# szpajder/dumpvdl2

Hardware: AMD Instinct MI355X
Metric: IQ MS/s demodulated end-to-end (higher is better)
Workload: dtype f32

## Files before the change

dumpvdl2_amd/csrc/debug_hooks.inc:

```

static bool hip_ok(hipError_t e) { return e == hipSuccess; }
template<typename T> static bool dbg_up(const DevBuf<T> &d, const void *src, size_t bytes) { return hip_ok(hipMemcpy(d, src, bytes, hipMemcpyHostToDevice)); }
template<typename T> static bool dbg_up(const DevBuf<T> &d, const void *src) { return dbg_up(d, src, d.bytes()); }
template<typename T> static bool dbg_fill(const DevBuf<T> &d, int v) { return hip_ok(hipMemset(d, v, d.bytes())); }
template<typename T> static bool dbg_down(void *dst, const DevBuf<T> &d, size_t bytes) { return hip_ok(hipMemcpy(dst, d, bytes, hipMemcpyDeviceToHost)); }
template<typename T> static bool dbg_down(void *dst, const DevBuf<T> &d) { return dbg_down(dst, d, d.bytes()); }
static bool dbg_tables(const DevBuf<Tables> &d) { auto tab = std::make_unique<Tables>(); build_tables(*tab); return dbg_up(d, tab.get()); }

template<int K> static int prof_read(const void *symbol, unsigned long long *out, int reset) {
	unsigned long long h[64][K];
	if(hipMemcpyFromSymbol(h, symbol, sizeof h) != hipSuccess) return -3;
	for(int k = 0; k < K; k++) { out[k] = 0; for(int s = 0; s < 64; s++) out[k] += h[s][k]; }
	if(reset) { memset(h, 0, sizeof h); if(hipMemcpyToSymbol(symbol, h, sizeof h) != hipSuccess) return -3; }
	return 0;
}

extern "C" {

int vdl2hip_debug_live_resources(long long out[3]) {
	if(!out) return VDL2HIP_E_INVAL;
	for(int i = 0; i < 3; i++) out[i] = hostmem::g_live[i].load();
	return VDL2HIP_OK;
}

int vdl2hip_debug_option(vdl2hip_ctx *c, const char *name, long value) {
	if(!c || !name) return VDL2HIP_E_INVAL;
	OnDevice dev_guard(c);
	int r = collect_pending(c);
	if(r != VDL2HIP_OK && r != VDL2HIP_E_OVERFLOW) return r;
	if(strcmp(name, "no_fuse") == 0) { c->fuse_k2 = value == 0; return VDL2HIP_OK; }
	if(strcmp(name, "force_timeout") == 0) { c->debug_force_timeout = value != 0; return VDL2HIP_OK; }
	if(strcmp(name, "force_mismatch") == 0) { c->debug_force_mismatch = value != 0; return VDL2HIP_OK; }
	if(strcmp(name, "walk_ahead_below") == 0) { c->walk_ahead_below = (double)value; c->walk_ahead_auto = true; return VDL2HIP_OK; }
	if(strcmp(name, "mark_cap") == 0) { if(value < 0 || value > (long long)kDeferScansMax) return VDL2HIP_E_INVAL; c->debug_mark_cap = (uint32_t)value; return VDL2HIP_OK; }
	if(strcmp(name, "walk_ahead") == 0) { if(value != 0 && value != 1) return VDL2HIP_E_INVAL; c->walk_ahead = (int)value; c->walk_ahead_auto = false; return VDL2HIP_OK; }
	if(strcmp(name, "exact_tier") == 0) { if(value != 0 && value != 1) return VDL2HIP_E_INVAL; c->debug_exact_tier = (int)value; return VDL2HIP_OK; }
	if(strcmp(name, "screen_all") == 0) { c->debug_screen_all = value != 0; return VDL2HIP_OK; }
	if(strcmp(name, "force_again") == 0) { c->debug_force_again = value != 0; return VDL2HIP_OK; }
	if(strcmp(name, "referee") == 0) { if(value && !c->d_refhist) return VDL2HIP_E_INVAL; c->referee = value != 0; return VDL2HIP_OK; }
	if(strcmp(name, "ref_warm") == 0) { if(value < 0 || value > c->ref_T - 4096) return VDL2HIP_E_INVAL; c->ref_warm = value; return VDL2HIP_OK; }
	return VDL2HIP_E_INVAL;
}

int vdl2hip_debug_exact_window_many(vdl2hip_ctx *c, uint32_t chan, int64_t n_lo, int64_t n_hi, uint32_t count, int64_t stride, float *ms) {
	if(!c || !c->d_refhist || chan >= (uint32_t)c->C || c->feed_no == 0 || count == 0 || count > 65536) return VDL2HIP_E_INVAL;
	OnDevice dev_guard(c);
	int r = collect_pending(c);
	if(r != VDL2HIP_OK && r != VDL2HIP_E_OVERFLOW) return r;
	DevBuf<int> d_out; std::vector<int> h(count, 0);
	if(!hip_ok(d_out.alloc(count))) return VDL2HIP_E_NOMEM;
	Event e0, e1;
	if(!hip_ok(e0.ensure()) || !hip_ok(e1.ensure())) return VDL2HIP_E_DEVICE;
	hipExtLaunchKernelGGL(k_ref_probe, dim3(count), dim3(64), 0, c->streams.front, e0, e1, 0, c->d_ref[(c->feed_no - 1) % kSlots].get(), (int)chan, c->C, n_lo, n_hi, stride, d_out.get());
	if(!hip_ok(hipStreamSynchronize(c->streams.front)) || !dbg_down(h.data(), d_out)) return VDL2HIP_E_DEVICE;
	if(ms) { float t = 0.f; (void)hipEventElapsedTime(&t, e0, e1); *ms = t; }
	int n = 0; for(int v : h) n += v;
	return n;
}
int vdl2hip_debug_scan_multi2(vdl2hip_ctx *c, const int32_t *chan, const int64_t *lo, const int64_t *hi, uint32_t count, int with_retry, float *ms) {
	if(!c || !c->d_refhist || c->feed_no == 0 || count == 0 || count > 65536 || !chan || !lo || !hi) return VDL2HIP_E_INVAL;
	OnDevice dev_guard(c);
	int r = collect_pending(c);
	if(r != VDL2HIP_OK && r != VDL2HIP_E_OVERFLOW) return r;
	std::vector<ScanReq> h(count);
	for(uint32_t i = 0; i < count; i++) { if(chan[i] < 0 || chan[i] >= c->C) return VDL2HIP_E_INVAL; h[i] = ScanReq{ chan[i], REF_CANDIDATE, lo[i], hi[i] }; }
	DevBuf<ScanReq> d_sq, d_rt; DevBuf<uint32_t> d_n;
	if(!hip_ok(d_sq.alloc(count)) || !hip_ok(d_n.alloc(2)) || !hip_ok(d_rt.alloc(kRetryScans))) return VDL2HIP_E_NOMEM;
	uint32_t before[8] = {0}, after[8] = {0};
	const uint32_t nn[2] = { count, 0u };
	Event e0, e1;
	if(!hip_ok(e0.ensure()) || !hip_ok(e1.ensure()) || !dbg_up(d_sq, h.data()) || !dbg_up(d_n, nn) || !dbg_down(before, c->d_refstats, sizeof before)) return VDL2HIP_E_DEVICE;
	RefChan *ref = c->d_ref[(c->feed_no - 1) % kSlots];
	launch_scans(c, c->streams.front, ref, 0xfffeu, d_sq, nullptr, d_n, count, c->k_total, with_retry ? d_rt.get() : nullptr, d_n + 1, e0, e1);
	if(!hip_ok(hipStreamSynchronize(c->streams.front)) || !dbg_down(after, c->d_refstats, sizeof after)) return VDL2HIP_E_DEVICE;
	if(ms) { float t = 0.f; (void)hipEventElapsedTime(&t, e0, e1); *ms = t; }
	return (int)(after[0] - before[0]);
}
int vdl2hip_debug_exact_window(vdl2hip_ctx *c, uint32_t chan, int64_t n_lo, int64_t n_hi) { return vdl2hip_debug_exact_window_many(c, chan, n_lo, n_hi, 1, 0, nullptr); }

int vdl2hip_debug_u8_levels(float out[512]) {
	DevBuf<float> d;
	if(!hip_ok(d.alloc(512))) return VDL2HIP_E_NOMEM;
	hipLaunchKernelGGL(k_u8_level_probe, dim3(1), dim3(256), 0, 0, d);
	return dbg_down(out, d) ? VDL2HIP_OK : VDL2HIP_E_DEVICE;
}

int vdl2hip_debug_s8_levels(float out[512]) {
	DevBuf<float> d;
	if(!hip_ok(d.alloc(512))) return VDL2HIP_E_NOMEM;
// ... 466 lines not shown
```

dumpvdl2_amd/csrc/kernels.h:

```cpp
#pragma once
#include <hip/hip_runtime.h>
#include <type_traits>
#include "vdl2_core.h"
#include "design.h"

#ifndef VDL2_K1_UNROLL
#define VDL2_K1_UNROLL 5
#endif

#ifndef VDL2_K1_WAVES_PER_EU
#define VDL2_K1_WAVES_PER_EU 3
#endif

namespace vdl2 {

constexpr int kK1Unroll = VDL2_K1_UNROLL;
typedef float v2f __attribute__((ext_vector_type(2)));
typedef float v4f __attribute__((ext_vector_type(4)));

#ifndef VDL2_REF_PRIO
#define VDL2_REF_PRIO 3
#endif
#ifndef VDL2_K1_PRIO
#define VDL2_K1_PRIO 0
// ... 902 lines not shown
	const int c = blockIdx.y;
	if(k >= a.D) return;
	const BlockForm &bf = *a.bf;
	const uint32_t slot = (uint32_t)(a.k0 + k) & a.mask;
	const int seg = (int)(k / a.seglen), i = (int)(k - (int64_t)seg * a.seglen);
	if(i < kFixW) {
		cf32 v = a.y[(size_t)c * a.cap + slot];
		const float4 ts = seg ? a.seg_end[(size_t)c * a.nseg_cap + seg - 1] : a.carry_in[c];
		v.re += bf.cP[i][0] * ts.x + bf.cP[i][1] * ts.z;
		v.im += bf.cP[i][0] * ts.y + bf.cP[i][1] * ts.w;
		a.y[(size_t)c * a.cap + slot] = v;
	}
	if(k == a.D - 1) {
		const int len = i + 1;
		float4 e = a.seg_end[(size_t)c * a.nseg_cap + seg];
		if(len <= kFixW) {
			const float4 ts = seg ? a.seg_end[(size_t)c * a.nseg_cap + seg - 1] : a.carry_in[c];
			const float *Pp = bf.Ppow[len];
			e.x += Pp[0] * ts.x + Pp[1] * ts.z; e.y += Pp[0] * ts.y + Pp[1] * ts.w;
			e.z += Pp[2] * ts.x + Pp[3] * ts.z; e.w += Pp[2] * ts.y + Pp[3] * ts.w;
		}
		a.carry_out[c] = e;
	}
}

__global__ void k_carry(K1Args a, void *carry_out, uint32_t nrem) {
	const uint32_t i = threadIdx.x;
	if(i >= nrem) return;
	const int64_t s = (int64_t)(a.nlogical - nrem) + i;
	if(a.fmt == 2) {
		const uint2 *p = (s < (int64_t)a.ncarry) ? (const uint2 *)a.carry + s : (const uint2 *)a.in + (s - a.ncarry);
		((uint2 *)carry_out)[i] = *p;
	} else if(a.fmt == 1) {
		const uint32_t *p = (s < (int64_t)a.ncarry) ? (const uint32_t *)a.carry + s : (const uint32_t *)a.in + (s - a.ncarry);
		((uint32_t *)carry_out)[i] = *p;
	} else {
		const uint16_t *p = (s < (int64_t)a.ncarry) ? (const uint16_t *)a.carry + s : (const uint16_t *)a.in + (s - a.ncarry);
		((uint16_t *)carry_out)[i] = *p;
	}
}

__device__ __forceinline__ void reset_out_ctl(OutCtl *ctl, uint32_t k5_waves) {
	ctl->nbursts = 0; ctl->overflow = 0; ctl->nvalid = 0; ctl->pool_out_used = 0;
	ctl->nframes = burst_reserve_initial_frames(k5_waves); ctl->pool_used = burst_reserve_initial_pool(k5_waves);
}
__global__ void k_reset_ctl(OutCtl *ctl, uint32_t k5_waves) { reset_out_ctl(ctl, k5_waves); }

struct K3Args {
	const cf32 *y; cf32 *pf; uint64_t *cand; uint64_t *flag; const Tables *tab;
	int64_t nbase, k1;
	uint32_t cap, mask;
	int32_t wpl;
	int32_t screen_all;
	OutCtl *ctl; uint32_t k5_waves;
	RefChan *ref; RefChan refv; float max_ppm; const float *ppm_thr; int32_t ref_on; uint32_t *rq_n, *rq_flag; RefBad *rq_bad; ScanReq *pq; uint32_t pq_cap; uint32_t *rq_flag2;
};

#ifndef VDL2_K3_SHARE
#define VDL2_K3_SHARE 8
#endif
constexpr int kK3Share = VDL2_K3_SHARE, kK3Threads = 320, kK3Tile = kK3Threads * kK3Share;
static_assert(kK3Tile == kK3Threads * kK3Share && kK3Tile % 64 == 0 && kK3Threads % 10 == 0 && (kK3Tile / 64) % (kK3Threads / 64) == 0, "screen tile");

__global__ __launch_bounds__(kK3Threads) void k_sync_screen(K3Args a) {
	if(blockIdx.x == 0 && blockIdx.y == 0 && threadIdx.x == 0 && a.rq_n) a.rq_n[3] = 0u;
	__shared__ float tile[kK3Tile + 150];
	__shared__ uint8_t verdict[kK3Tile];
	const int c = blockIdx.y, tid = threadIdx.x;
	const int64_t nblk = a.nbase + (int64_t)blockIdx.x * kK3Tile;
	const cf32 *y = a.y + (size_t)c * a.cap;
	constexpr int kFull = (kK3Tile + 150) / kK3Threads, kRest = (kK3Tile + 150) % kK3Threads;
	const bool full_tile = nblk >= 150 && nblk + kK3Tile <= a.k1;
	if(full_tile) {
		const uint32_t r0 = (uint32_t)(nblk - 150) + tid;
		cf32 v[kFull + 1];
		#pragma unroll
		for(int k = 0; k <= kFull; k++) if(k < kFull || tid < kRest) v[k] = y[(r0 + kK3Threads * k) & a.mask];
		#pragma unroll
		for(int k = 0; k <= kFull; k++) if(k < kFull || tid < kRest) tile[tid + kK3Threads * k] = phase_fast(v[k]);
	} else {
		for(int j = tid; j < kK3Tile + 150; j += kK3Threads) {
			const int64_t t = nblk - 150 + j;
			tile[j] = (t < 0 || t >= a.k1) ? 0.f : phase_fast(y[(uint32_t)t & a.mask]);
		}
	}
	__syncthreads();
	const int s0 = 10 * kK3Share * (tid / 10) + tid % 10;
	constexpr int kEarlyPh = kScreenEarly + kK3Share - 1;
	float ph[kEarlyPh], d[kEarlyPh];
	#pragma unroll
	for(int k = 0; k < kEarlyPh; k++) ph[k] = tile[s0 + 10 * k];
	#pragma unroll
	for(int k = 1; k < kEarlyPh; k++) d[k] = ph[k] - ph[k - 1];
	#pragma unroll
	for(int q = 0; q < kK3Share; q++) {
		ScreenAcc acc;
		screen_begin(acc);
		screen_taps(&d[q], 1, kScreenEarly, acc);
		float ps = screen_value(acc, kScreenEarly);
		if(__any(ps < kScreenEarlyThr)) {
			float pl[kPreamble - kScreenEarly + 1], dl[kPreamble];
			#pragma unroll
			for(int j = 0; j <= kPreamble - kScreenEarly; j++) pl[j] = tile[s0 + 10 * (q + kScreenEarly - 1 + j)];
			#pragma unroll
			for(int j = 0; j < kPreamble - kScreenEarly; j++) dl[kScreenEarly + j] = pl[j + 1] - pl[j];
			screen_taps(dl, kScreenEarly, kPreamble, acc);
// ... 131 lines not shown
			#pragma unroll
			for(int k = 0; k < 4; k++) if(64 * k + lane < kSpan) e2[64 * k + lane] = ev[k];
			WAVE_SYNC();
		}
		K3B_MARK(2);
		#pragma unroll 1
		for(int round = 0; round < 2; round++) {
			const int bit = round == 0 ? lane : lane - 6;
			const bool todo = round == 0 ? ((needj >> lane) & 1ull) != 0 : (lane < 6 && ((fprevj >> lane) & 1u) && (wj << 6) + bit >= 0);
			if(todo) {
				const int i0 = bit + kBack - 150;
				float p[kPreamble];
				#pragma unroll
				for(int i = 0; i < kPreamble; i++) p[i] = ph[i0 + 10 * i];
				float pv, fv, E = 0.f, pa, pb;
				if(ref_on) sync_metric_ref(p, e2 + i0, 10, T, pv, fv, E, pa, pb, FULL);
				else { sync_metric(p, T, pv, fv); pa = pb = pv; }
				ps[6 + bit] = pv; fs[6 + bit] = fv; es[6 + bit] = E; as[6 + bit] = pa; bs[6 + bit] = pb;
			}
			K3B_MARK(3 + round);
		}
		WAVE_SYNC();
		const int64_t n = (wj << 6) + lane;
		const float p0 = ps[6 + lane], p3 = ps[3 + lane], p6 = ps[lane];
		int vd = 0;
		if(n >= 3 && n < a.k1) {
			if(!ref_on) vd = is_candidate(p3, p0) ? 1 : 0;
			else vd = ref_candidate_verdict(ref_pherr_range(p0, as[6 + lane], bs[6 + lane], es[6 + lane]), ref_pherr_range(p3, as[3 + lane], bs[3 + lane], es[3 + lane]), fs[3 + lane], es[3 + lane],
			                                ref_pherr_range(p6, as[lane], bs[lane], es[lane]), a.max_ppm, ppm_thr);
		}
		if((needj >> lane) & 1ull) a.pf[(size_t)c * a.cap + ((uint32_t)n & a.mask)] = cf32{ (vd & 2) ? -p0 : p0, fs[6 + lane] };
		const unsigned long long bits = __ballot((vd & 1) != 0);
		if(lane == 0) cand[(uint32_t)wj & wmask] = bits;
		if(a.pq) {
			const unsigned long long mk = __ballot((vd & 2) != 0 && ((needj >> lane) & 1ull) != 0);
			if(mk && lane == 0) {
				const int64_t nf = (wj << 6) + __builtin_ctzll(mk), nl = (wj << 6) + 63 - __builtin_clzll(mk);
				int64_t lo = (nf - kRefPre) & ~255ll, hi = (nl + kRefPost) | 255; if(lo < 0) lo = 0; if(hi > a.k1 - 1) hi = a.k1 - 1;
				const uint32_t i = atomicAdd(a.rq_n + 3, 1u);
				if(i < a.pq_cap) a.pq[i] = ScanReq{ c, REF_CANDIDATE, lo, hi };
			}
		}
		WAVE_SYNC();
		K3B_MARK(5);
	}
	K3B_END();
}

constexpr int kK3dEvals = 320;
constexpr int kK3dFlush = kK3dEvals - 64;
constexpr int kK3dList = kK3dFlush + 256;
constexpr int kK3dMinGroups = 2048;
constexpr int kK3dGroup = 4;
constexpr int kK3dRounds = 32;
static_assert(kK3dEvals >= 70 && kK3dEvals <= 512 && kK3dList * 70 < (1 << 20) && kK3dList < (1 << 11) && kK3dRounds * 256 <= (1 << 16),
              "tile map: 9 bits of word, 7 of position; list head: 11 bits of words, 21 of evaluations; 16 bits of word index");
#define K3D_BARRIER() do { __builtin_amdgcn_fence(__ATOMIC_RELEASE, "workgroup", "local"); __builtin_amdgcn_s_barrier(); __builtin_amdgcn_fence(__ATOMIC_ACQUIRE, "workgroup", "local"); } while(0)
template<bool FULL>
__global__ __launch_bounds__(256, 4) void k_sync_dense(K3Args a) {
	if(blockIdx.x == 0 && blockIdx.y == 0 && threadIdx.x == 0) { reset_out_ctl(a.ctl, a.k5_waves); if(a.ref) *a.ref = a.refv; if(a.rq_n) { a.rq_n[0] = 0u; a.rq_n[1] = 0u; a.rq_n[2] = 0u; a.rq_n[4] = 0u; a.rq_n[5] = 0u; a.rq_n[6] = 0u; a.rq_n[7] = 0u; } }
	if(blockIdx.x == 0 && threadIdx.x == 0 && a.rq_flag) { a.rq_flag[blockIdx.y] = 0u; a.rq_bad[blockIdx.y].n = 0u; if(a.rq_flag2) a.rq_flag2[blockIdx.y] = 0u; }
	__shared__ uint64_t s_need[kK3dList], s_cbits[kK3dList], s_mbits[kK3dList];
	__shared__ uint32_t s_end[kK3dList];
	__shared__ uint16_t s_word[kK3dList];
	__shared__ uint8_t s_fprev[kK3dList];
	__shared__ uint16_t s_map[kK3dEvals];
	__shared__ float s_res[5][kK3dEvals];
	__shared__ uint8_t s_neg[kK3dEvals];
	__shared__ uint32_t s_head, s_r1;
	__shared__ uint64_t s_flag[256 * kK3dGroup + 3];
	const int c = blockIdx.y, tid = threadIdx.x, lane = threadIdx.x & 63;
	const cf32 *y = a.y + (size_t)c * a.cap;
	const uint64_t *flag = a.flag + (size_t)c * (a.cap >> 6);
	uint64_t *cand = a.cand + (size_t)c * (a.cap >> 6);
	const uint32_t wmask = a.mask >> 6;
	const Tables &T = *a.tab;
	const bool ref_on = a.ref != nullptr && a.ref_on != 0;
	const float ppm_thr = ref_on ? a.ppm_thr[c] : 0.f;
	const int64_t w0 = a.nbase >> 6, w1 = (a.k1 + 63) >> 6;
	const int64_t wb = w0 + (int64_t)blockIdx.x * (256 * a.wpl);
	K3B_BEGIN();
	if(tid == 0) s_head = 0u;
	K3D_BARRIER();
	#pragma unroll 1
	for(int g = 0; g < a.wpl; g++) {
		if(g % kK3dGroup == 0) {
			const int ng = a.wpl - g < kK3dGroup ? a.wpl - g : kK3dGroup;
			for(int i = tid; i < 256 * ng + 3; i += 256) {
				const int64_t w = wb + 256 * g - 2 + i;
				s_flag[i] = w >= 0 && w < w1 ? flag[(uint32_t)w & wmask] : 0ull;
			}
			K3D_BARRIER();
		}
		{
			const int64_t w = wb + 256 * g + tid;
			const int fi = 256 * (g % kK3dGroup) + tid;
			uint64_t need = 0, fprev = 0, fpp = 0, f0 = 0;
			if(w < w1) {
				f0 = s_flag[fi + 2]; fprev = s_flag[fi + 1]; fpp = s_flag[fi];
				const uint64_t fnext = s_flag[fi + 3];
				need = f0 | (f0 << 3) | (f0 >> 3) | (fprev >> 61) | (fnext << 61);
				const int64_t base = w << 6;
				if(a.k1 - 3 < base + 64) {
					const int64_t lo = a.k1 - 3 - base;
					need |= lo <= 0 ? ~0ull : (~0ull << lo);
				}
				if(a.k1 < base + 64) need &= (a.k1 - base <= 0) ? 0ull : (~0ull >> (64 - (a.k1 - base)));
				if(need == 0) cand[(uint32_t)w & wmask] = 0;
			}
			const uint64_t need_prev = fprev | (fprev << 3) | (fprev >> 3) | (fpp >> 61) | (f0 << 61);
			const uint32_t fp6 = w > 0 ? (uint32_t)(need_prev >> 58) : 0u;
			const uint32_t cnt = need != 0 ? (uint32_t)__builtin_popcountll(need) + (uint32_t)__builtin_popcount(fp6) : 0u;
			const uint32_t inc = cnt << 11 | (need != 0 ? 1u : 0u);
			uint32_t incl = inc;
			#pragma unroll
			for(int d = 1; d < 64; d <<= 1) { const uint32_t o = (uint32_t)__shfl_up((int)incl, d); if(lane >= d) incl += o; }
			const uint32_t tot = (uint32_t)__shfl((int)incl, 63);
			uint32_t at = 0;
			if(lane == 0 && tot != 0) at = atomicAdd(&s_head, tot);
			at = (uint32_t)__shfl((int)at, 0) + incl - inc;
			if(need != 0) {
				const uint32_t r = at & 2047u;
				s_need[r] = need; s_fprev[r] = (uint8_t)fp6; s_word[r] = (uint16_t)(256 * g + tid); s_end[r] = (at >> 11) + cnt;
				s_cbits[r] = 0ull; s_mbits[r] = 0ull;
			}
		}
		K3D_BARRIER();
		const uint32_t head = s_head;
		K3D_BARRIER();
		const int nrec = (int)(head & 2047u);
		K3B_MARK(0);
		if((int)(head >> 11) < kK3dFlush && g + 1 < a.wpl) continue;
		K3B_COUNT(0, nrec); K3B_COUNT(1, head >> 11);
		#pragma unroll 1
		for(int r0 = 0; r0 < nrec; ) {
			const uint32_t e0 = r0 ? s_end[r0 - 1] : 0u;
			if(tid == 0) s_r1 = (uint32_t)r0 + 1u;
			K3D_BARRIER();
			{
				uint32_t best = 0;
				for(int r = r0 + 1 + tid; r < nrec && r < r0 + kK3dEvals; r += 256) if(s_end[r] - e0 <= (uint32_t)kK3dEvals) best = (uint32_t)r + 1u;
				if(best) atomicMax(&s_r1, best);
			}
			K3D_BARRIER();
			const int r1 = (int)s_r1, nev = (int)(s_end[r1 - 1] - e0);
			for(int r = r0 + tid; r < r1; r += 256) {
				uint32_t at = (r ? s_end[r - 1] : 0u) - e0;
				const uint32_t code = (uint32_t)(r - r0) << 7;
				for(uint32_t m = s_fprev[r]; m; m &= m - 1u) s_map[at++] = (uint16_t)(code | (uint32_t)__builtin_ctz(m));
				for(uint64_t m = s_need[r]; m; m &= m - 1ull) s_map[at++] = (uint16_t)(code | (6u + (uint32_t)__builtin_ctzll(m)));
			}
			K3D_BARRIER();
			K3B_MARK(1); K3B_COUNT(2, 1);
			#pragma unroll 1
			for(int s = tid; s < nev; s += 256) {
				const uint32_t code = s_map[s];
				const int64_t n = ((wb + s_word[r0 + (int)(code >> 7)]) << 6) + (int)(code & 127u) - 6;
				float p[kPreamble], e2[kPreamble];
				cf32 yt[kPreamble];
				#pragma unroll
				for(int i = 0; i < kPreamble; i++) { const int64_t t = n - 150 + 10 * i; yt[i] = t >= 0 ? y[(uint32_t)t & a.mask] : cf32{0.f, 0.f}; }
				if(ref_on) {
					#pragma unroll
					for(int h = 0; h < kPreamble; h += 4) {
						cf32 yv[4][3];
						#pragma unroll
						for(int i = 0; i < 4; i++) {
							#pragma unroll
							for(int k = 0; k < 3; k++) { const int64_t t = n - 150 + 10 * (h + i) - 1 - k; yv[i][k] = t >= 0 ? y[(uint32_t)t & a.mask] : cf32{0.f, 0.f}; }
						}
						#pragma unroll
						for(int i = 0; i < 4; i++) {
							const int64_t t = n - 150 + 10 * (h + i);
							float m[4];
							m[0] = t >= 0 ? yt[h + i].re * yt[h + i].re + yt[h + i].im * yt[h + i].im : -1.f;
							#pragma unroll
							for(int k = 0; k < 3; k++) m[1 + k] = t - 1 - k >= 0 ? yv[i][k].re * yv[i][k].re + yv[i][k].im * yv[i][k].im : -1.f;
							e2[h + i] = m[0] < 0.f ? 0.f : ref_eps2_of(m[0], fmaxf(m[1], 0.f), fmaxf(m[2], 0.f), fmaxf(m[3], 0.f));
						}
					}
				}
				#pragma unroll
				for(int i = 0; i < kPreamble; i++) { const int64_t t = n - 150 + 10 * i; p[i] = t >= 0 ? phase_of(yt[i]) : 0.f; }
				float pv, fv, E = 0.f, pa, pb;
				if(ref_on) sync_metric_ref(p, e2, 1, T, pv, fv, E, pa, pb, FULL);
				else { sync_metric(p, T, pv, fv); pa = pb = pv; }
				s_res[0][s] = pv; s_res[1][s] = fv; s_res[2][s] = E; s_res[3][s] = pa; s_res[4][s] = pb; s_neg[s] = 0;
			}
			K3D_BARRIER();
			K3B_MARK(3);
			#pragma unroll 1
			for(int s = tid; s < nev; s += 256) {
				const uint32_t code = s_map[s];
				const int r = r0 + (int)(code >> 7), pos = (int)(code & 127u) + 3;
				if(pos < 6 || pos > 69) continue;
				const uint64_t needj = s_need[r];
				const uint64_t mlo = (uint64_t)s_fprev[r] | (needj << 6), mhi = needj >> 58;
				const int at = (int)((r ? s_end[r - 1] : 0u) - e0);
// ... 784 lines not shown
```

dumpvdl2_amd/csrc/vdl2hip.hip:

```cpp
#include <hip/hip_runtime.h>
#include <hip/hip_ext.h>
#include <algorithm>
#include <cmath>
#include <cstddef>
#include <cstdio>
#include <cstdlib>
#include <cstring>
#include <deque>
#include <map>
#include <memory>
#include <mutex>
#include <new>
#include <string>
#include <vector>
#include "../../include/vdl2hip.h"
#include "kernels.h"
#include "resample.h"
#include "resample_design.h"
#include "spectrum.h"
#include "spectrum_design.h"
#include "activity.h"
#include "txlog.h"
#include "txsearch.h"
#include "capture.h"
// ... 111 lines not shown
	struct {
		bool on = false; uint32_t B = 0, H = 0, S = 0; float thr_dbfs = 0.f, thr = 0.f; int64_t k_on = 0; uint64_t bins = 0;
		struct { DevBuf<float> d_series, d_carry[2], d_edges; DevBuf<ActChan> d_acc; DevBuf<ActState> d_st; } buf;
		int carry_sel = 0; TapRead tap; double kernel_ms = 0.0;
	} act;
	struct CapItem { vdl2hip_burst r; std::shared_ptr<std::vector<float>> iq; };
	struct {
		bool on = false; uint32_t pre = 0, post = 0, flags = 0, pool = 0;
		uint64_t bursts = 0, iq_samples = 0, iq_dropped = 0; double kernel_ms = 0.0;
		PinnedBuf stage;
		std::deque<CapItem> queue;
	} capt;
	struct TxFrame { int64_t sync_sample, burst_ord; bool ok; };
	struct {
		bool on = false; uint32_t pool = 0, flags = 0;
		uint64_t transmissions = 0, decoded = 0, dropped = 0, matched = 0, unmatched = 0; double kernel_ms = 0.0;
		struct { DevBuf<TxState> d_st; DevBuf<uint32_t> d_cnt; PinnedBuf stage; } buf;
		std::deque<vdl2hip_tx> queue; std::vector<std::deque<TxFrame>> wait;
	} txl;
	struct {
		bool on = false; uint32_t flags = 0, piece_cap = 0;
		uint64_t records = 0, samples = 0, clipped = 0; double kernel_ms = 0.0;
		PinnedBuf stage; std::deque<vdl2hip_tx_search> queue;
	} txs;
	uint64_t dmax = 0;
	bool specialised = false;
	std::vector<uint32_t> freqs, dphi, all_freqs;
	LpfCoeffs lpf{};
	BlockForm bf{};
	StreamSet streams;
	DevBuf<BlockForm> d_bf; DevBuf<Lut4> d_lut; DevBuf<Tables> d_tab;
	DevBuf<uint32_t> d_dphi, d_freq; DevBuf<float> d_ppmthr;
	DevBuf<uint8_t> d_in[kSlots]; Event ev_copied[kSlots]; size_t in_cap = 0;
	hipEvent_t pinned_pending = nullptr;
	struct { int n = 0; uint64_t samples[kColdParts] = {}; Event ev[kColdParts]; } cold;
	PinnedBuf stage;
	DevBuf<uint8_t> d_carry[2]; int carry_sel = 0; uint32_t ncarry = 0;
	DevBuf<cf32> d_y, d_pf; DevBuf<uint64_t> d_cand, d_flag;
	uint32_t cap = 0;
	DevBuf<float4> d_segend; uint32_t nseg_cap = 0;
	DevBuf<float4> d_qpow;
	DevBuf<float4> d_tcarry[2]; int tcarry_sel = 0;
	DevBuf<unsigned long long> d_segpub; DevBuf<uint32_t> d_synctmo; bool fuse_k2 = true;
	DevBuf<WalkState> d_ws; DevBuf<unsigned long long> d_cnt, d_acnt;
	unsigned long long *d_wcnt = nullptr;
	DevBuf<NfState> d_nf; DevBuf<int64_t> d_scfirst, d_sccum;
	DevBuf<float> d_nfring, d_lpbuf; DevBuf<NfFeed> d_nffeed; uint32_t cap_log = 0, cap_comb = 0, cap_hist = 0, nf_ring = 0;
	uint32_t cap_bursts_chan = 0;
	DevBuf<SpecOut> d_spec[2]; DevBuf<uint32_t> d_segstats; int seg_max = 1; int64_t seg_min = 16384;
	OutSlot slot[kSlots];
	uint64_t feed_no = 0; int drain_lag = 0;
	OutCtl ctl_template{};
	bool pooled = false;
	bool avlc_filter = false, failed = false; int debug_force_timeout = 0, debug_force_again = 0, debug_exact_tier = 1, debug_screen_all = 0;
	bool referee = true; bool ref_prescan = false;    int64_t ref_warm = 3 << 16 , ref_T = 0; DevBuf<uint8_t> d_refhist; uint64_t ref_cap = 0, ref_wp = 0;
	struct HistPiece { int64_t s0, n; uint64_t pos; }; std::vector<HistPiece> ref_pieces;
	DevBuf<WalkState> d_ws_snap[2], d_ws_tmp; DevBuf<unsigned long long> d_cnt_snap[2], d_cnt_tmp; uint32_t rq_cap = 8192; uint32_t sq_alloc = 8192;
	int walk_ahead = 1; bool walk_ahead_auto = true; double walk_ahead_below = 1.1e8; int debug_force_mismatch = 0; uint32_t debug_mark_cap = 0;
	int ref_retry_mul = 2;
	DevBuf<RefChan> d_ref[kSlots]; DevBuf<unsigned long long> d_refdone; DevBuf<uint32_t> d_refdonen, d_refstats; DevBuf<uint8_t> d_mix;
	std::vector<uint64_t> statsd_prev;
	std::vector<HostFrame> queue;
	int64_t k_total = 0; uint64_t n_total = 0;
	int profiling = 0;
	vdl2hip_stats stats{};
};

#define HIPCHK(expr) do { hipError_t e_ = (expr); if(e_ != hipSuccess) { \
	fprintf(stderr, "vdl2hip: %s failed: %s (%s:%d)\n", #expr, hipGetErrorString(e_), __FILE__, __LINE__); return VDL2HIP_E_DEVICE; } } while(0)

constexpr int kFmtS8 = 3;
static int fmt_code(uint32_t sample_fmt) {
	switch(sample_fmt) {
		case VDL2HIP_FMT_U8: case VDL2HIP_FMT_S16LE: case VDL2HIP_FMT_CF32: return (int)sample_fmt;
		case VDL2HIP_FMT_S8: return kFmtS8;
		default: return -1;
	}
}
static size_t sample_bytes(int fmt) { return fmt == VDL2HIP_FMT_CF32 ? 8 : fmt == VDL2HIP_FMT_S16LE ? 4 : 2; }

struct OnDevice {
	int prev = -1; bool switched = false;
	explicit OnDevice(const vdl2hip_ctx *c) { if(c && hipGetDevice(&prev) == hipSuccess && prev != c->cfg.device) switched = hipSetDevice(c->cfg.device) == hipSuccess; }
	~OnDevice() { if(switched) (void)hipSetDevice(prev); }
};

#define LAUNCH_EV(kernel, grid, block, stream, e0, e1, ...) hipExtLaunchKernelGGL(kernel, grid, block, 0u, stream, e0, e1, 0, __VA_ARGS__)
#define EV(i) (prof_all ? (hipEvent_t)ev[i] : (hipEvent_t) nullptr)

template<int OS, int R>
static void launch_chanfir(vdl2hip_ctx *c, const K1Args &a, int cr, size_t lds, hipEvent_t e0, hipEvent_t e1) {
	const int groups = (c->C + cr - 1) / cr;
	K1Args b = a;
	b.gy = (groups + 3) / 4;
	const int nseg8 = (a.seg1 - a.seg0 + 7) / 8 * 8;
	dim3 grid((unsigned)(nseg8 * b.gy)), block(256);
	if(c->fmt == VDL2HIP_FMT_CF32) {
		switch(cr) {
			case 4: hipExtLaunchKernelGGL((k_chanfir<OS, R, 4, false, true>), grid, block, (uint32_t)lds, c->streams.front, e0, e1, 0, b); break;
			case 2: hipExtLaunchKernelGGL((k_chanfir<OS, R, 2, false, true>), grid, block, (uint32_t)lds, c->streams.front, e0, e1, 0, b); break;
			default: hipExtLaunchKernelGGL((k_chanfir<OS, R, 1, false, true>), grid, block, (uint32_t)lds, c->streams.front, e0, e1, 0, b); break;
		}
		return;
	}
	switch(cr) {
		case 4:
			if constexpr(OS == 20 || OS == 10) { if(c->fmt == VDL2HIP_FMT_U8) { hipExtLaunchKernelGGL((k_chanfir<OS, R, 4, true>), grid, block, (uint32_t)lds, c->streams.front, e0, e1, 0, b); break; } }
// ... 187 lines not shown
				if(p < c->cold.n - 1) { const uint64_t r = (c->ncarry + c->cold.samples[p]) / seg_in; ready = r >= (uint64_t)a.nseg ? a.nseg : (int)(r & ~7ull); }
				if(ready > done) { launch(done, ready, done == 0 ? e0 : (hipEvent_t) nullptr, ready == a.nseg ? e1 : (hipEvent_t) nullptr); done = ready; }
			}
		}
		if(!a.fuse) {
			K2Args k2{ c->d_y, c->d_segend, c->d_tcarry[c->tcarry_sel], c->d_tcarry[c->tcarry_sel ^ 1], c->d_bf,
			           c->k_total, D, c->cap, c->cap - 1, c->nseg_cap, seglen * a.tiles };
			LAUNCH_EV(k_fixup, dim3((unsigned)((D + 255) / 256), (unsigned)c->C), dim3(256), st, EV(2), EV(3), k2);
		}
		c->tcarry_sel ^= 1;
		if(c->act.on) { int r = activity_feed(c, sl, c->k_total, D); if(r != VDL2HIP_OK) return r; }
	}
	if(nrem) hipLaunchKernelGGL(k_carry, dim3(1), dim3(64), 0, st, a, (void *)c->d_carry[c->carry_sel ^ 1], nrem);
	c->carry_sel ^= 1; c->ncarry = nrem;
	RefChan refv{}; RefChan *ref_dst = nullptr;
	if(c->d_refhist) {
		ref_dst = c->d_ref[c->feed_no % kSlots];
		refv.y = c->d_y; refv.cap = c->cap; refv.mask = c->cap - 1; refv.dphi = c->d_dphi; refv.mix = c->d_mix; refv.lut = c->d_lut;
		refv.A0 = c->lpf.A[0]; refv.A1 = c->lpf.A[1]; refv.A2 = c->lpf.A[2]; refv.B1 = c->lpf.B[1]; refv.B2 = c->lpf.B[2];
		refv.os = c->os; refv.fmt = c->fmt; refv.warm = c->ref_warm;
		refv.done = c->d_refdone; refv.done_n = c->d_refdonen; refv.stats = c->d_refstats;
		int np = 0;
		const int64_t blk_s0 = (int64_t)c->n_total, want0 = blk_s0 - c->ref_T;
		for(size_t i = c->ref_pieces.size() > 2 ? c->ref_pieces.size() - 2 : 0; i < c->ref_pieces.size(); i++) {
			vdl2hip_ctx::HistPiece hp = c->ref_pieces[i];
			if(hp.s0 + hp.n <= want0) continue;
			if(hp.s0 < want0) { hp.pos = (hp.pos + (uint64_t)(want0 - hp.s0)) % c->ref_cap; hp.n -= want0 - hp.s0; hp.s0 = want0; }
			const uint64_t first = std::min<uint64_t>((uint64_t)hp.n, c->ref_cap - hp.pos);
			refv.piece[np++] = RefPiece{ c->d_refhist + hp.pos * sb, hp.s0, (int64_t)first };
			if(first < (uint64_t)hp.n) refv.piece[np++] = RefPiece{ c->d_refhist, hp.s0 + (int64_t)first, hp.n - (int64_t)first };
		}
		refv.piece[np++] = RefPiece{ dev_in, blk_s0, (int64_t)nnew };
		refv.npiece = np;
		int firstp = 0;
		for(int i = 1; i < np; i++) if(refv.piece[i - 1].s0 + refv.piece[i - 1].n != refv.piece[i].s0) firstp = i;
		if(firstp) { for(int i = firstp; i < np; i++) refv.piece[i - firstp] = refv.piece[i]; refv.npiece = np - firstp; }
		if(nnew) {
			const uint64_t w = std::min<uint64_t>(nnew, (uint64_t)c->ref_T);
			hipLaunchKernelGGL(k_ref_hist, dim3((unsigned)((w + 255) / 256)), dim3(256), 0, st, (const uint8_t *)dev_in + (nnew - w) * sb, w, c->d_refhist, c->ref_wp, c->ref_cap, (int)sb);
			if(w < nnew) c->ref_pieces.clear();
			if(!c->ref_pieces.empty() && c->ref_pieces.back().s0 + c->ref_pieces.back().n == blk_s0 + (int64_t)(nnew - w)) c->ref_pieces.back().n += (int64_t)w;
			else c->ref_pieces.push_back(vdl2hip_ctx::HistPiece{ blk_s0 + (int64_t)(nnew - w), (int64_t)w, c->ref_wp });
			c->ref_wp = (c->ref_wp + w) % c->ref_cap;
			auto &bp = c->ref_pieces.back();
			if((uint64_t)bp.n > c->ref_cap / 2) { const int64_t cut = bp.n - (int64_t)(c->ref_cap / 2); bp.s0 += cut; bp.pos = (bp.pos + (uint64_t)cut) % c->ref_cap; bp.n -= cut; }
			while(c->ref_pieces.size() > 2) c->ref_pieces.erase(c->ref_pieces.begin());
		}
	}
	if(D > 0) {
		const int64_t k1 = c->k_total + D, nbase = c->k_total & ~63ll;
		sl.k5_waves = (unsigned)std::min<int64_t>(2048, std::max<int64_t>(16, (D * (int64_t)c->C) >> 14));
		sl.k5_waves = (sl.k5_waves + kBurstWaves - 1) / kBurstWaves * kBurstWaves;
		sl.prescan = c->referee && c->ref_prescan && !feed_is_small(c, D);
		K3Args k3{ c->d_y, c->d_pf, c->d_cand, c->d_flag, c->d_tab, nbase, k1, c->cap, c->cap - 1, 1, c->debug_screen_all, sl.d_ctl, sl.k5_waves, ref_dst, refv, c->cfg.max_ppm, c->d_ppmthr, c->referee ? 1 : 0, sl.d_rqn, sl.d_rqflag, sl.d_rqbad, sl.prescan ? sl.d_pq : nullptr, kPreScans, sl.d_rqflag2 };
		LAUNCH_EV(k_sync_screen, dim3((unsigned)((k1 - nbase + kK3Tile - 1) / kK3Tile), (unsigned)c->C), dim3(kK3Threads), st, EV(4), (hipEvent_t) nullptr, k3);
		const int64_t nwords = ((k1 + 63) >> 6) - (nbase >> 6);
		for(int wpl = kK3bWordsPerLane; wpl >= 1; wpl >>= 1) { k3.wpl = wpl; if(((nwords + 256 * wpl - 1) / (256 * wpl)) * c->C >= 2048 || wpl == 1) break; }
		if(c->debug_exact_tier) {
			for(int wpl = kK3dRounds; wpl >= 1; wpl >>= 1) { k3.wpl = wpl; if(((nwords + 256 * wpl - 1) / (256 * wpl)) * c->C >= kK3dMinGroups || wpl == 1) break; }
		}
		const int64_t wpb = 256 * k3.wpl;
		const dim3 k3b_grid((unsigned)((nwords + wpb - 1) / wpb), (unsigned)c->C);
		if(c->debug_exact_tier) {
			if(c->referee && c->ref_prescan) LAUNCH_EV(k_sync_dense<true>, k3b_grid, dim3(256), st, (hipEvent_t) nullptr, sl.ev_front, k3);
			else LAUNCH_EV(k_sync_dense<false>, k3b_grid, dim3(256), st, (hipEvent_t) nullptr, sl.ev_front, k3);
		} else {
			if(c->referee && c->ref_prescan) LAUNCH_EV(k_sync_exact4<true>, k3b_grid, dim3(256), st, (hipEvent_t) nullptr, sl.ev_front, k3);
			else LAUNCH_EV(k_sync_exact4<false>, k3b_grid, dim3(256), st, (hipEvent_t) nullptr, sl.ev_front, k3);
		}
	}
	if(D <= 0) HIPCHK(hipEventRecord(sl.ev_front, st));
	if(D > 0) { sl.ev_valid = prof; sl.ev_level = c->profiling; sl.fused = a.fuse != 0; if(sl.k1_timed) c->stats.chan_samples += (uint64_t)D * c->os * c->C; } else sl.k1_timed = false;
	sl.back_D = D; sl.back_k0 = c->k_total;
	sl.pending = true; sl.seq = c->feed_no++;
	c->k_total += D; c->n_total += nnew;
	c->stats.feeds++; c->stats.input_samples += nnew;
	{ int r = launch_back(c, sl); if(r != VDL2HIP_OK) return r; }
	HIPCHK(hipGetLastError());
	return VDL2HIP_OK;
}

template<int FMT>
static void launch_resample(vdl2hip_ctx *c, const K0Args &a, unsigned grid, hipEvent_t e0, hipEvent_t e1) {
	if(c->rs.taps_lds) hipExtLaunchKernelGGL((k_resample<FMT, true>), dim3(grid), dim3(kResTile), (uint32_t)c->rs.lds, c->streams.front, e0, e1, 0, a);
	else hipExtLaunchKernelGGL((k_resample<FMT, false>), dim3(grid), dim3(kResTile), (uint32_t)c->rs.lds, c->streams.front, e0, e1, 0, a);
}
static int monitor_block(vdl2hip_ctx *c, const void *dev_in, size_t nbytes);
static int feed_block(vdl2hip_ctx *c, const void *dev_in, size_t nbytes, bool in_parts = false) {
	if(c->failed) return VDL2HIP_E_DEVICE;
	if(!c->rs.on) {
		if(c->mon.on) { int r = monitor_block(c, dev_in, nbytes); if(r != VDL2HIP_OK) return r; }
		return feed_common(c, dev_in, nbytes, in_parts);
	}
	auto &rs = c->rs;
	const int k = (int)(c->feed_no % kSlots);
	OutSlot &sl = c->slot[k];
	{ int r = collect_slot(c, sl); if(r != VDL2HIP_OK && r != VDL2HIP_E_OVERFLOW) return r; }
	const uint64_t nin = nbytes / sample_bytes(c->in_fmt);
	const uint64_t N0 = rs.n_in, N1 = N0 + nin, n0 = rs.n_out, n1 = (N1 * rs.L + rs.M - 1) / rs.M, nout = n1 - n0;
	if(nout > rs.cap) return VDL2HIP_E_TOOBIG;
	if(c->mon.on) { int r = monitor_block(c, dev_in, nbytes); if(r != VDL2HIP_OK) return r; }
	K0Args a{};
	a.in = dev_in; a.tail_in = rs.d_tail[rs.tail_sel]; a.tail_out = rs.d_tail[rs.tail_sel ^ 1]; a.taps = rs.d_taps; a.out = rs.d_out[k];
	a.q0 = n0 % rs.L; a.t0 = n0 * rs.M - N0 * rs.L;
	a.nin = (uint32_t)nin; a.nout = (uint32_t)nout; a.L = rs.L; a.M = rs.M; a.T = rs.T; a.span_cap = rs.span_cap;
	const uint64_t per = (uint64_t)kResTile * kResTiles;
	const unsigned grid = (unsigned)std::max<uint64_t>(1, (nout + per - 1) / per);
	KernelTimes &t = sl.rs_t;
	t.arm(c->profiling >= 2);
	if(c->in_fmt == VDL2HIP_FMT_CF32) launch_resample<2>(c, a, grid, t.e(0), t.e(1));
	else if(c->in_fmt == VDL2HIP_FMT_S16LE) launch_resample<1>(c, a, grid, t.e(0), t.e(1));
	else if(c->in_fmt == kFmtS8) launch_resample<3>(c, a, grid, t.e(0), t.e(1));
// ... 1423 lines not shown
```

Baseline: 5779.

## Add single-pass sparse fast path to dense sync kernel list building

```diff
diff --git a/dev/gpu_k3b_phases.py b/dev/gpu_k3b_phases.py
--- /dev/null
+++ b/dev/gpu_k3b_phases.py
@@ -0,0 +1,25 @@
+import ctypes, os, sys
+sys.path.insert(0, os.path.dirname(os.path.dirname(os.path.abspath(__file__))))
+import numpy as np
+from dumpvdl2_amd import vdl2hip, synth, workloads
+L = vdl2hip.load_library(os.environ['VDL2HIP_LIB'])
+cfg = workloads.config4(float(sys.argv[1]) if len(sys.argv) > 1 else 16.0)
+iq, _ = synth.synthesize(cfg, workers=8)
+raw = np.ascontiguousarray(iq).view(np.uint8).reshape(-1)
+rx = vdl2hip.Receiver(cfg.centerfreq, list(cfg.freqs), cfg.oversample, vdl2hip.FMT_S16LE, cfg.rx_max_ppm, max_block_bytes=raw.size)
+a = (ctypes.c_ulonglong * 16)()
+for _ in range(2):
+    rx.feed(raw); rx.drain()
+L.vdl2hip_debug_k3b_prof(a, 1)
+reps = 3
+for _ in range(reps):
+    rx.feed(raw); rx.drain()
+L.vdl2hip_debug_k3b_prof(a, 0)
+names = ["list", "tile set-up", "count (sparse case)", "evaluate", "-", "decide + stores"]
+wgs = a[8] or 1
+tot = sum(a[k] for k in range(6))
+print(f"{os.path.basename(os.environ['VDL2HIP_LIB'])}: {wgs // reps} workgroups a feed; {a[9] / wgs:.1f} busy words, {a[10] / wgs:.1f} evaluations, {a[11] / wgs:.2f} tiles per workgroup; shader clocks of wave 0 per workgroup")
+for k in (2, 0, 1, 3, 5):
+    print(f"  {names[k]:20s} {a[k] / wgs:9.0f} {100.0 * a[k] / tot:5.1f} %")
+print(f"  {'total':20s} {tot / wgs:9.0f}")
+rx.close()
diff --git a/dumpvdl2_amd/csrc/debug_hooks.inc b/dumpvdl2_amd/csrc/debug_hooks.inc
--- a/dumpvdl2_amd/csrc/debug_hooks.inc
+++ b/dumpvdl2_amd/csrc/debug_hooks.inc
@@ -35,6 +35,8 @@
 	if(strcmp(name, "mark_cap") == 0) { if(value < 0 || value > (long long)kDeferScansMax) return VDL2HIP_E_INVAL; c->debug_mark_cap = (uint32_t)value; return VDL2HIP_OK; }
 	if(strcmp(name, "walk_ahead") == 0) { if(value != 0 && value != 1) return VDL2HIP_E_INVAL; c->walk_ahead = (int)value; c->walk_ahead_auto = false; return VDL2HIP_OK; }
 	if(strcmp(name, "exact_tier") == 0) { if(value != 0 && value != 1) return VDL2HIP_E_INVAL; c->debug_exact_tier = (int)value; return VDL2HIP_OK; }
+	if(strcmp(name, "dense_fast") == 0) { if(value != 0 && value != 1) return VDL2HIP_E_INVAL; c->debug_dense_fast = (int)value; return VDL2HIP_OK; }
+	if(strcmp(name, "dense_passes") == 0) { if(value < 0 || value > kK3dRounds) return VDL2HIP_E_INVAL; c->debug_dense_passes = (int)value; return VDL2HIP_OK; }
 	if(strcmp(name, "screen_all") == 0) { c->debug_screen_all = value != 0; return VDL2HIP_OK; }
 	if(strcmp(name, "force_again") == 0) { c->debug_force_again = value != 0; return VDL2HIP_OK; }
 	if(strcmp(name, "referee") == 0) { if(value && !c->d_refhist) return VDL2HIP_E_INVAL; c->referee = value != 0; return VDL2HIP_OK; }
diff --git a/dumpvdl2_amd/csrc/kernels.h b/dumpvdl2_amd/csrc/kernels.h
--- a/dumpvdl2_amd/csrc/kernels.h
+++ b/dumpvdl2_amd/csrc/kernels.h
@@ -978,6 +978,7 @@
 	uint32_t cap, mask;
 	int32_t wpl;
 	int32_t screen_all;
+	int32_t dense_fast;
 	OutCtl *ctl; uint32_t k5_waves;
 	RefChan *ref; RefChan refv; float max_ppm; const float *ppm_thr; int32_t ref_on; uint32_t *rq_n, *rq_flag; RefBad *rq_bad; ScanReq *pq; uint32_t pq_cap; uint32_t *rq_flag2;
 };
@@ -1215,9 +1216,33 @@
 constexpr int kK3dList = kK3dFlush + 256;
 constexpr int kK3dMinGroups = 2048;
 constexpr int kK3dGroup = 4;
+constexpr int kK3dFast = 8;
 constexpr int kK3dRounds = 32;
+static_assert(kK3dFast % kK3dGroup == 0 && 6 * kK3dFast <= 64 && kK3dFast <= kK3dRounds, "the sparse case: whole groups of flag fetches, six bits a pass in one word");
 static_assert(kK3dEvals >= 70 && kK3dEvals <= 512 && kK3dList * 70 < (1 << 20) && kK3dList < (1 << 11) && kK3dRounds * 256 <= (1 << 16),
               "tile map: 9 bits of word, 7 of position; list head: 11 bits of words, 21 of evaluations; 16 bits of word index");
+__device__ __forceinline__ void k3d_flags(const uint64_t *flag, uint32_t wmask, int64_t w, int64_t w1, uint64_t f[4]) {
+	#pragma unroll
+	for(int i = 0; i < 4; i++) f[i] = flag[(uint32_t)(w - 2 + i) & wmask];
+	#pragma unroll
+	for(int i = 0; i < 4; i++) { const int64_t x = w - 2 + i; if(!(w < w1 && x >= 0 && x < w1)) f[i] = 0ull; }
+}
+__device__ __forceinline__ uint32_t k3d_word_work(const uint64_t f[4], int64_t w, int64_t w1, int64_t k1, uint64_t &need, uint32_t &fp6) {
+	need = 0; fp6 = 0u;
+	if(!(w < w1)) return 0u;
+	const uint64_t fpp = f[0], fprev = f[1], f0 = f[2], fnext = f[3];
+	need = f0 | (f0 << 3) | (f0 >> 3) | (fprev >> 61) | (fnext << 61);
+	const int64_t base = w << 6;
+	if(k1 - 3 < base + 64) {
+		const int64_t lo = k1 - 3 - base;
+		need |= lo <= 0 ? ~0ull : (~0ull << lo);
+	}
+	if(k1 < base + 64) need &= (k1 - base <= 0) ? 0ull : (~0ull >> (64 - (k1 - base)));
+	if(need == 0) return 0u;
+	const uint64_t need_prev = fprev | (fprev << 3) | (fprev >> 3) | (fpp >> 61) | (f0 << 61);
+	fp6 = w > 0 ? (uint32_t)(need_prev >> 58) : 0u;
+	return ((uint32_t)__builtin_popcountll(need) + (uint32_t)__builtin_popcount(fp6)) << 11 | 1u;
+}
 #define K3D_BARRIER() do { __builtin_amdgcn_fence(__ATOMIC_RELEASE, "workgroup", "local"); __builtin_amdgcn_s_barrier(); __builtin_amdgcn_fence(__ATOMIC_ACQUIRE, "workgroup", "local"); } while(0)
 template<bool FULL>
 __global__ __launch_bounds__(256, 4) void k_sync_dense(K3Args a) {
@@ -1230,7 +1255,7 @@
 	__shared__ uint16_t s_map[kK3dEvals];
 	__shared__ float s_res[5][kK3dEvals];
 	__shared__ uint8_t s_neg[kK3dEvals];
-	__shared__ uint32_t s_head, s_r1;
+	__shared__ uint32_t s_head, s_r1, s_wtot[4];
 	__shared__ uint64_t s_flag[256 * kK3dGroup + 3];
 	const int c = blockIdx.y, tid = threadIdx.x, lane = threadIdx.x & 63;
 	const cf32 *y = a.y + (size_t)c * a.cap;
@@ -1244,53 +1269,104 @@
 	const int64_t wb = w0 + (int64_t)blockIdx.x * (256 * a.wpl);
 	K3B_BEGIN();
 	if(tid == 0) s_head = 0u;
+	uint32_t fast_at = 0u, fast_tot = 0u;
+	uint64_t fneed[kK3dFast], ffp6 = 0ull;
+	const bool try_fast = a.dense_fast && a.wpl <= kK3dFast;
+	if(try_fast) {
+		uint32_t mine = 0u;
+		#pragma unroll
+		for(int g0 = 0; g0 < kK3dFast; g0 += kK3dGroup) {
+			uint64_t f[kK3dGroup][4];
+			if(g0 < a.wpl) {
+				#pragma unroll
+				for(int k = 0; k < kK3dGroup; k++) k3d_flags(flag, wmask, wb + 256 * (g0 + k) + tid, g0 + k < a.wpl ? w1 : 0, f[k]);
+			}
+			#pragma unroll
+			for(int k = 0; k < kK3dGroup; k++) {
+				uint32_t fp6 = 0u;
+				fneed[g0 + k] = 0ull;
+				if(g0 < a.wpl) mine += k3d_word_work(f[k], wb + 256 * (g0 + k) + tid, g0 + k < a.wpl ? w1 : 0, a.k1, fneed[g0 + k], fp6);
+				ffp6 |= (uint64_t)fp6 << (6 * (g0 + k));
+			}
+		}
+		uint32_t incl = mine;
+		#pragma unroll
+		for(int d = 1; d < 64; d <<= 1) { const uint32_t o = (uint32_t)__shfl_up((int)incl, d); if(lane >= d) incl += o; }
+		if(lane == 63) s_wtot[tid >> 6] = incl;
+		fast_at = incl - mine;
+	}
 	K3D_BARRIER();
+	if(try_fast) {
+		#pragma unroll
+		for(int k = 0; k < 4; k++) { const uint32_t t = s_wtot[k]; fast_tot += t; if(k < (tid >> 6)) fast_at += t; }
+	}
+	K3B_MARK(2);
+	const bool fast = try_fast && (fast_tot >> 11) <= (uint32_t)kK3dEvals && (fast_tot & 2047u) <= (uint32_t)kK3dList;
+	if(fast) {
+		#pragma unroll
+		for(int g = 0; g < kK3dFast; g++) {
+			const int64_t w = wb + 256 * g + tid;
+			const uint64_t need = fneed[g];
+			if(g < a.wpl && w < w1 && need == 0) cand[(uint32_t)w & wmask] = 0;
+			if(need != 0) {
+				const uint32_t fp6 = (uint32_t)(ffp6 >> (6 * g)) & 63u, cnt = (uint32_t)__builtin_popcountll(need) + (uint32_t)__builtin_popcount(fp6);
+				const uint32_t r = fast_at & 2047u;
+				s_need[r] = need; s_fprev[r] = (uint8_t)fp6; s_word[r] = (uint16_t)(256 * g + tid); s_end[r] = (fast_at >> 11) + cnt;
+				s_cbits[r] = 0ull; s_mbits[r] = 0ull;
+				fast_at += cnt << 11 | 1u;
+			}
+		}
+		K3D_BARRIER();
+	}
 	#pragma unroll 1
-	for(int g = 0; g < a.wpl; g++) {
-		if(g % kK3dGroup == 0) {
-			const int ng = a.wpl - g < kK3dGroup ? a.wpl - g : kK3dGroup;
-			for(int i = tid; i < 256 * ng + 3; i += 256) {
-				const int64_t w = wb + 256 * g - 2 + i;
-				s_flag[i] = w >= 0 && w < w1 ? flag[(uint32_t)w & wmask] : 0ull;
+	for(int g = fast ? a.wpl - 1 : 0; g < a.wpl; g++) {
+		uint32_t head = fast_tot;
+		if(!fast) {
+			if(g % kK3dGroup == 0) {
+				const int ng = a.wpl - g < kK3dGroup ? a.wpl - g : kK3dGroup;
+				for(int i = tid; i < 256 * ng + 3; i += 256) {
+					const int64_t w = wb + 256 * g - 2 + i;
+					s_flag[i] = w >= 0 && w < w1 ? flag[(uint32_t)w & wmask] : 0ull;
+				}
+				K3D_BARRIER();
+			}
+			{
+				const int64_t w = wb + 256 * g + tid;
+				const int fi = 256 * (g % kK3dGroup) + tid;
+				uint64_t need = 0, fprev = 0, fpp = 0, f0 = 0;
+				if(w < w1) {
+					f0 = s_flag[fi + 2]; fprev = s_flag[fi + 1]; fpp = s_flag[fi];
+					const uint64_t fnext = s_flag[fi + 3];
+					need = f0 | (f0 << 3) | (f0 >> 3) | (fprev >> 61) | (fnext << 61);
+					const int64_t base = w << 6;
+					if(a.k1 - 3 < base + 64) {
+						const int64_t lo = a.k1 - 3 - base;
+						need |= lo <= 0 ? ~0ull : (~0ull << lo);
+					}
+					if(a.k1 < base + 64) need &= (a.k1 - base <= 0) ? 0ull : (~0ull >> (64 - (a.k1 - base)));
+					if(need == 0) cand[(uint32_t)w & wmask] = 0;
+				}
+				const uint64_t need_prev = fprev | (fprev << 3) | (fprev >> 3) | (fpp >> 61) | (f0 << 61);
+				const uint32_t fp6 = w > 0 ? (uint32_t)(need_prev >> 58) : 0u;
+				const uint32_t cnt = need != 0 ? (uint32_t)__builtin_popcountll(need) + (uint32_t)__builtin_popcount(fp6) : 0u;
+				const uint32_t inc = cnt << 11 | (need != 0 ? 1u : 0u);
+				uint32_t incl = inc;
+				#pragma unroll
+				for(int d = 1; d < 64; d <<= 1) { const uint32_t o = (uint32_t)__shfl_up((int)incl, d); if(lane >= d) incl += o; }
+				const uint32_t tot = (uint32_t)__shfl((int)incl, 63);
+				uint32_t at = 0;
+				if(lane == 0 && tot != 0) at = atomicAdd(&s_head, tot);
+				at = (uint32_t)__shfl((int)at, 0) + incl - inc;
+				if(need != 0) {
+					const uint32_t r = at & 2047u;
+					s_need[r] = need; s_fprev[r] = (uint8_t)fp6; s_word[r] = (uint16_t)(256 * g + tid); s_end[r] = (at >> 11) + cnt;
+					s_cbits[r] = 0ull; s_mbits[r] = 0ull;
+				}
 			}
 			K3D_BARRIER();
-		}
-		{
-			const int64_t w = wb + 256 * g + tid;
-			const int fi = 256 * (g % kK3dGroup) + tid;
-			uint64_t need = 0, fprev = 0, fpp = 0, f0 = 0;
-			if(w < w1) {
-				f0 = s_flag[fi + 2]; fprev = s_flag[fi + 1]; fpp = s_flag[fi];
-				const uint64_t fnext = s_flag[fi + 3];
-				need = f0 | (f0 << 3) | (f0 >> 3) | (fprev >> 61) | (fnext << 61);
-				const int64_t base = w << 6;
-				if(a.k1 - 3 < base + 64) {
-					const int64_t lo = a.k1 - 3 - base;
-					need |= lo <= 0 ? ~0ull : (~0ull << lo);
-				}
-				if(a.k1 < base + 64) need &= (a.k1 - base <= 0) ? 0ull : (~0ull >> (64 - (a.k1 - base)));
-				if(need == 0) cand[(uint32_t)w & wmask] = 0;
-			}
-			const uint64_t need_prev = fprev | (fprev << 3) | (fprev >> 3) | (fpp >> 61) | (f0 << 61);
-			const uint32_t fp6 = w > 0 ? (uint32_t)(need_prev >> 58) : 0u;
-			const uint32_t cnt = need != 0 ? (uint32_t)__builtin_popcountll(need) + (uint32_t)__builtin_popcount(fp6) : 0u;
-			const uint32_t inc = cnt << 11 | (need != 0 ? 1u : 0u);
-			uint32_t incl = inc;
-			#pragma unroll
-			for(int d = 1; d < 64; d <<= 1) { const uint32_t o = (uint32_t)__shfl_up((int)incl, d); if(lane >= d) incl += o; }
-			const uint32_t tot = (uint32_t)__shfl((int)incl, 63);
-			uint32_t at = 0;
-			if(lane == 0 && tot != 0) at = atomicAdd(&s_head, tot);
-			at = (uint32_t)__shfl((int)at, 0) + incl - inc;
-			if(need != 0) {
-				const uint32_t r = at & 2047u;
-				s_need[r] = need; s_fprev[r] = (uint8_t)fp6; s_word[r] = (uint16_t)(256 * g + tid); s_end[r] = (at >> 11) + cnt;
-				s_cbits[r] = 0ull; s_mbits[r] = 0ull;
-			}
-		}
-		K3D_BARRIER();
-		const uint32_t head = s_head;
-		K3D_BARRIER();
+			head = s_head;
+			K3D_BARRIER();
+		}
 		const int nrec = (int)(head & 2047u);
 		K3B_MARK(0);
 		if((int)(head >> 11) < kK3dFlush && g + 1 < a.wpl) continue;
@@ -1298,15 +1374,17 @@
 		#pragma unroll 1
 		for(int r0 = 0; r0 < nrec; ) {
 			const uint32_t e0 = r0 ? s_end[r0 - 1] : 0u;
-			if(tid == 0) s_r1 = (uint32_t)r0 + 1u;
-			K3D_BARRIER();
-			{
-				uint32_t best = 0;
-				for(int r = r0 + 1 + tid; r < nrec && r < r0 + kK3dEvals; r += 256) if(s_end[r] - e0 <= (uint32_t)kK3dEvals) best = (uint32_t)r + 1u;
-				if(best) atomicMax(&s_r1, best);
-			}
-			K3D_BARRIER();
-			const int r1 = (int)s_r1, nev = (int)(s_end[r1 - 1] - e0);
+			if(!fast) {
+				if(tid == 0) s_r1 = (uint32_t)r0 + 1u;
+				K3D_BARRIER();
+				{
+					uint32_t best = 0;
+					for(int r = r0 + 1 + tid; r < nrec && r < r0 + kK3dEvals; r += 256) if(s_end[r] - e0 <= (uint32_t)kK3dEvals) best = (uint32_t)r + 1u;
+					if(best) atomicMax(&s_r1, best);
+				}
+				K3D_BARRIER();
+			}
+			const int r1 = fast ? nrec : (int)s_r1, nev = (int)(s_end[r1 - 1] - e0);
 			for(int r = r0 + tid; r < r1; r += 256) {
 				uint32_t at = (r ? s_end[r - 1] : 0u) - e0;
 				const uint32_t code = (uint32_t)(r - r0) << 7;
diff --git a/dumpvdl2_amd/csrc/vdl2hip.hip b/dumpvdl2_amd/csrc/vdl2hip.hip
--- a/dumpvdl2_amd/csrc/vdl2hip.hip
+++ b/dumpvdl2_amd/csrc/vdl2hip.hip
@@ -187,7 +187,7 @@
 	uint64_t feed_no = 0; int drain_lag = 0;
 	OutCtl ctl_template{};
 	bool pooled = false;
-	bool avlc_filter = false, failed = false; int debug_force_timeout = 0, debug_force_again = 0, debug_exact_tier = 1, debug_screen_all = 0;
+	bool avlc_filter = false, failed = false; int debug_force_timeout = 0, debug_force_again = 0, debug_exact_tier = 1, debug_screen_all = 0, debug_dense_fast = 1, debug_dense_passes = 0;
 	bool referee = true; bool ref_prescan = false;    int64_t ref_warm = 3 << 16 , ref_T = 0; DevBuf<uint8_t> d_refhist; uint64_t ref_cap = 0, ref_wp = 0;
 	struct HistPiece { int64_t s0, n; uint64_t pos; }; std::vector<HistPiece> ref_pieces;
 	DevBuf<WalkState> d_ws_snap[2], d_ws_tmp; DevBuf<unsigned long long> d_cnt_snap[2], d_cnt_tmp; uint32_t rq_cap = 8192; uint32_t sq_alloc = 8192;
@@ -481,12 +481,13 @@
 		sl.k5_waves = (unsigned)std::min<int64_t>(2048, std::max<int64_t>(16, (D * (int64_t)c->C) >> 14));
 		sl.k5_waves = (sl.k5_waves + kBurstWaves - 1) / kBurstWaves * kBurstWaves;
 		sl.prescan = c->referee && c->ref_prescan && !feed_is_small(c, D);
-		K3Args k3{ c->d_y, c->d_pf, c->d_cand, c->d_flag, c->d_tab, nbase, k1, c->cap, c->cap - 1, 1, c->debug_screen_all, sl.d_ctl, sl.k5_waves, ref_dst, refv, c->cfg.max_ppm, c->d_ppmthr, c->referee ? 1 : 0, sl.d_rqn, sl.d_rqflag, sl.d_rqbad, sl.prescan ? sl.d_pq : nullptr, kPreScans, sl.d_rqflag2 };
+		K3Args k3{ c->d_y, c->d_pf, c->d_cand, c->d_flag, c->d_tab, nbase, k1, c->cap, c->cap - 1, 1, c->debug_screen_all, c->debug_dense_fast, sl.d_ctl, sl.k5_waves, ref_dst, refv, c->cfg.max_ppm, c->d_ppmthr, c->referee ? 1 : 0, sl.d_rqn, sl.d_rqflag, sl.d_rqbad, sl.prescan ? sl.d_pq : nullptr, kPreScans, sl.d_rqflag2 };
 		LAUNCH_EV(k_sync_screen, dim3((unsigned)((k1 - nbase + kK3Tile - 1) / kK3Tile), (unsigned)c->C), dim3(kK3Threads), st, EV(4), (hipEvent_t) nullptr, k3);
 		const int64_t nwords = ((k1 + 63) >> 6) - (nbase >> 6);
 		for(int wpl = kK3bWordsPerLane; wpl >= 1; wpl >>= 1) { k3.wpl = wpl; if(((nwords + 256 * wpl - 1) / (256 * wpl)) * c->C >= 2048 || wpl == 1) break; }
 		if(c->debug_exact_tier) {
 			for(int wpl = kK3dRounds; wpl >= 1; wpl >>= 1) { k3.wpl = wpl; if(((nwords + 256 * wpl - 1) / (256 * wpl)) * c->C >= kK3dMinGroups || wpl == 1) break; }
+			if(c->debug_dense_passes) k3.wpl = c->debug_dense_passes;
 		}
 		const int64_t wpb = 256 * k3.wpl;
 		const dim3 k3b_grid((unsigned)((nwords + wpb - 1) / wpb), (unsigned)c->C);
```

Result: no change. 5781, median of 2 (+0.0%).
